# malani86/unet-DC-segmentation

Measured on AMD Instinct MI355X. Metric: images/sec fwd+bwd, 512x512x1 U-Net-DC, bs=8/GPU, higher is better.
Workload: dtype bf16

## Files before the change

unet_dc_segmentation_amd/csrc/igemm_conv.hip:

```cpp
#include <stdlib.h>

#include <stdio.h>

#include "kernels.h"

namespace unetdc {

template <typename T> struct Mma;
template <> struct Mma<bf16_t> {
  __device__ static __forceinline__ void run(f32x16& acc, const u32x4& a, const u32x4& b) {
    acc = __builtin_amdgcn_mfma_f32_32x32x16_bf16(__builtin_bit_cast(bf16x8, a), __builtin_bit_cast(bf16x8, b),
                                                  acc, 0, 0, 0);
  }
};
template <> struct Mma<float> {
  __device__ static __forceinline__ void run(f32x16& acc, const u32x4& a, const u32x4& b) {
#pragma unroll
    for (int s = 0; s < 4; ++s) {
      const unsigned int ua = a[s], ub = b[s];
      acc = __builtin_amdgcn_mfma_f32_32x32x2f32(bits_f32(ua), bits_f32(ub), acc, 0, 0, 0);
    }
  }
};

// ... 187 lines not shown
    }
  }
  if (p.mode == MODE_STATS) {
    s0 += __shfl_xor(s0, 32, 64); q0 += __shfl_xor(q0, 32, 64);
    s1 += __shfl_xor(s1, 32, 64); q1 += __shfl_xor(q1, 32, 64);
    float* red = reinterpret_cast<float*>(smem);
    if (h == 0) {
      red[(wave * 4 + 0) * 32 + r] = s0;
      red[(wave * 4 + 1) * 32 + r] = q0;
      red[(wave * 4 + 2) * 32 + r] = s1;
      red[(wave * 4 + 3) * 32 + r] = q1;
    }
    __syncthreads();
    if (tid < BN) {
      const int wn2 = tid >> 6, c2 = tid & 63, r2 = c2 >> 1, e = c2 & 1;
      float su = 0.f, sq = 0.f;
#pragma unroll
      for (int w2 = 0; w2 < WM; ++w2) {
        su += red[((w2 * WN + wn2) * 4 + e * 2 + 0) * 32 + r2];
        sq += red[((w2 * WN + wn2) * 4 + e * 2 + 1) * 32 + r2];
      }
      p.stats[((long)mblk * 2 + 0) * p.Cout + n0 + tid] = su;
      p.stats[((long)mblk * 2 + 1) * p.Cout + n0 + tid] = sq;
    }
  }
}

int igemm_mblocks(long M, int Cout) { (void)Cout; return ceil_div(M, 256); }

template <typename T, int WM, int WN>
static int launch_cfg(IgemmParams& p, hipStream_t stream) {
  constexpr int BM = 64 * WM, BN = 64 * WN;
  constexpr int LDS = 2 * (BM + BN) * 128;
  if (const int rc_ = ensure_dynamic_lds(reinterpret_cast<const void*>(&igemm_conv_kernel<T, WM, WN>), LDS, "igemm_conv_kernel")) return rc_;
  p.mblocks = ceil_div(p.M, BM);
  p.nblocks = p.Cout / BN;
  const long nwg = (long)p.mblocks * p.nblocks;
  hipLaunchKernelGGL((igemm_conv_kernel<T, WM, WN>), dim3((unsigned)nwg), dim3(256), LDS, stream, p);
  char nm[96];
  snprintf(nm, sizeof(nm), "igemm_conv_kernel<%s, %d, %d>", sizeof(T) == 2 ? "__bf16" : "float", WM, WN);
  note_kernel(nm);
  return check_launch("igemm_conv_kernel");
}

IgemmPlan plan_igemm(const IgemmParams& p, int dtype) {
  IgemmPlan pl{};
  const bool lattice = igemm_lattice_supported(p, dtype);
  if (p.in_scale) {
    if (lattice && p.mode == MODE_STATS && (p.Cout % 128 == 0 || p.Cin <= 256)) {
      pl.route = IGEMM_LATTICE;
      pl.writes_act = p.Cout % 128 == 0 && (long)p.M * p.Cin * 2 < (1L << 32);
    }
    return pl;
  }
  if (lattice) {
    pl.route = IGEMM_LATTICE;
    return pl;
  }
  if (igemm_halo_supported(p, dtype)) {
    pl.route = IGEMM_HALO;
    return pl;
  }
  const long es = dtype == UNETDC_BF16 ? 2 : 4;
  const long HoWo = (long)p.Ho * p.Wo;
  const long xbytes = (p.M / HoWo) * p.Hi * p.Wi * p.ldx * es;
  const long wbytes = (long)p.ntaps * p.Cout * p.Cin * es;
  const long opix = p.mode == MODE_SHUFFLE ? 4L * p.M : (long)p.M;
  const long obytes = opix * p.ldo * es, ybytes = p.mode == MODE_BNBWD ? (long)p.M * p.bn_ldy * es : 0;
  if (!(xbytes < (1L << 31) && wbytes < (1L << 31) && obytes < (1L << 32) && ybytes < (1L << 32) && p.M % HoWo == 0)) {
    pl.route = IGEMM_FIRSTGEN;
    pl.cfg = (p.Cout % 128 == 0) && p.mode != MODE_STATS;
    return pl;
  }
  const long blocks_a = (long)((p.M + 255) / 256) * (p.Cout / 256);
  const bool use_a = p.Cout % 256 == 0 && p.M >= 256 * 64 && blocks_a >= 200;
  const bool use_b = !use_a && p.Cout % 128 == 0;
  pl.route = IGEMM_DMA;
  pl.cfg = use_a ? 1 : (use_b ? 2 : 3);
  if (dtype == UNETDC_BF16 && p.M % 16 == 0 && !(p.mode == MODE_SHUFFLE && p.Wo % 16 != 0)) {
    pl.route = IGEMM_DMA16;
    const long blocks_b = (long)((p.M + 255) / 256) * (p.Cout / 128);
    if (pl.cfg == 2 && p.mode == MODE_SHUFFLE && p.Cout % 256 == 0 && blocks_a >= 200) pl.cfg = 1;
    else if (pl.cfg == 2 && blocks_b >= 100 && blocks_b < 200) pl.cfg = 3;
  }
  return pl;
}

int launch_igemm(IgemmParams& p, int dtype, hipStream_t stream) {
  const int esz = dtype == UNETDC_BF16 ? 2 : 4;
  const int ke = 128 / esz;
  UNETDC_REQUIRE(dtype == UNETDC_F32 || dtype == UNETDC_BF16, "igemm: bad dtype %d", dtype);
  UNETDC_REQUIRE(p.x && p.w && p.out, "igemm: null tensor pointer");
  UNETDC_REQUIRE(p.M > 0 && p.Cin > 0 && p.Cout > 0, "igemm: empty problem");
  UNETDC_REQUIRE(p.Cin % ke == 0, "igemm: Cin=%d must be a multiple of %d for this dtype", p.Cin, ke);
  UNETDC_REQUIRE(p.Cout % 64 == 0, "igemm: Cout=%d must be a multiple of 64", p.Cout);
  UNETDC_REQUIRE(p.ldx % (16 / esz) == 0 && p.ldo % (16 / esz) == 0, "igemm: ld not 16-byte aligned");
  UNETDC_REQUIRE(((uintptr_t)p.x % 16 == 0) && ((uintptr_t)p.w % 16 == 0) && ((uintptr_t)p.out % 16 == 0),
                 "igemm: pointers must be 16-byte aligned");
  UNETDC_REQUIRE(p.ntaps >= 1 && p.ntaps <= 9, "igemm: ntaps out of range");
  UNETDC_REQUIRE((long)p.M < (1L << 31) - 512, "igemm: too many pixels");
  if (p.mode == MODE_SHUFFLE) UNETDC_REQUIRE(p.shuf_c % 64 == 0, "igemm: convT channels must be a multiple of 64");
  if (p.mode == MODE_STATS) UNETDC_REQUIRE(p.stats != nullptr, "igemm: stats buffer missing");
  if (p.mode == MODE_AFFINE_RELU) UNETDC_REQUIRE(p.scale && p.shift, "igemm: scale/shift missing");
  if (p.mode == MODE_BNBWD)
    UNETDC_REQUIRE(p.stats && p.bn_y && p.scale && p.shift && p.bn_mean && p.bn_rstd, "igemm: BN-backward inputs missing");
  {
    const long howo = (long)p.Ho * p.Wo;
    const bool p2 = (p.Wo & (p.Wo - 1)) == 0 && (howo & (howo - 1)) == 0;
    p.wo_shift = p2 ? __builtin_ctz((unsigned)p.Wo) : -1;
    p.howo_shift = p2 ? __builtin_ctzl((unsigned long)howo) : -1;
  }
  const IgemmPlan pl = plan_igemm(p, dtype);
  switch (pl.route) {
    case IGEMM_LATTICE: return launch_igemm_lattice(p, stream);
    case IGEMM_HALO: return launch_igemm_halo(p, dtype, stream);
    case IGEMM_DMA: return launch_igemm_dma(p, pl.cfg, dtype, stream);
    case IGEMM_DMA16: return launch_igemm_dma16(p, pl.cfg, stream);
    case IGEMM_FIRSTGEN:
      if (p.mode == MODE_BNBWD) {
        set_error("igemm: the first-generation kernel has no fused BatchNorm-backward sums");
        return UNETDC_EUNSUPPORTED;
      }
      if (dtype == UNETDC_BF16) return pl.cfg ? launch_cfg<bf16_t, 2, 2>(p, stream) : launch_cfg<bf16_t, 4, 1>(p, stream);
      return pl.cfg ? launch_cfg<float, 2, 2>(p, stream) : launch_cfg<float, 4, 1>(p, stream);
  }
  set_error("igemm: input normalisation asked for a shape / configuration the lattice kernel does not take");
  return UNETDC_EUNSUPPORTED;
}

}
```

unet_dc_segmentation_amd/csrc/igemm_dma16.hip:

```cpp
#include <stdio.h>
#include <stdlib.h>

#include "igemm_epilogue16.h"
#include "kernels.h"
#include "lds_dma.h"

namespace unetdc {

#define LDS_PTR16(p) ((__attribute__((address_space(3))) void*)(p))
constexpr unsigned OOB16 = 0x80000000u;

template <int WM, int WN, int TMT, int NS>
__global__ __launch_bounds__(512, 2) void igemm_dma16_kernel(const IgemmParams p) {
#if defined(__HIP_DEVICE_COMPILE__)
  constexpr int NW = WM * WN;
  constexpr int BM = WM * TMT * 16, BN = WN * 64;
  constexpr int AI = BM / 8 / NW, BI = BN / 8 / NW;
  constexpr int ES = 2, KE = 64;
  constexpr int STAGE = (BM + BN) * 128;
  constexpr int PER = AI + BI;
  static_assert(BM % (8 * NW) == 0 && BN % (8 * NW) == 0, "tile/wave mismatch");
  static_assert(NS == 2 || NS == 3, "ring depth");
  static_assert((NS - 2) * PER <= 63, "vmcnt is a 6-bit counter");
  extern __shared__ __attribute__((aligned(16))) unsigned char smem[];

  const int tid = threadIdx.x, lane = tid & 63;
  const int wave = __builtin_amdgcn_readfirstlane(tid >> 6);
  const int wm = wave / WN, wn = wave % WN;
  const int tile = xcd_remap(blockIdx.x, gridDim.x);
  const int mblk = tile / p.nblocks, nblk = tile - mblk * p.nblocks;
  const int m0 = mblk * BM, n0 = nblk * BN;
  const int HoWo = p.Ho * p.Wo;
  const unsigned lds_base = lds_addr_of(smem);

  const unsigned xbytes = (unsigned)(((long)p.M / HoWo) * p.Hi * p.Wi * p.ldx * ES);
  const unsigned wbytes = (unsigned)((long)p.ntaps * p.Cout * p.Cin * ES);
  const __amdgpu_buffer_rsrc_t xr = __builtin_amdgcn_make_buffer_rsrc(const_cast<void*>(p.x), 0, xbytes, 0x00020000);
  const __amdgpu_buffer_rsrc_t wr = __builtin_amdgcn_make_buffer_rsrc(const_cast<void*>(p.w), 0, wbytes, 0x00020000);

  const bool p2 = p.wo_shift >= 0;
  const bool quad = p.quad_bpr > 0;
  auto decode = [&](int m, int& n, int& oy, int& ox) {
    if (quad) {
      const int blk = m >> 8, r = m & 255;
      n = blk / p.quad_bpi;
      const int b = blk - n * p.quad_bpi;
      const int qy = b / p.quad_bpr;
      oy = qy * 16 + (r >> 4);
      ox = (b - qy * p.quad_bpr) * 16 + (r & 15);
    } else if (p2) {
      n = m >> p.howo_shift;
      const int rem = m & (HoWo - 1);
      oy = rem >> p.wo_shift;
      ox = rem & (p.Wo - 1);
    } else {
      n = m / HoWo;
      const int rem = m - n * HoWo;
      oy = rem / p.Wo;
      ox = rem - oy * p.Wo;
    }
  };
  unsigned tapmask = 0;
  {
    int na, ya, xa, nb, yb, xb;
    const int mlast = (m0 + BM < p.M ? m0 + BM : p.M) - 1;
    decode(m0, na, ya, xa);
    decode(mlast, nb, yb, xb);
    int by0 = 0, by1 = p.Ho - 1, bx0 = 0, bx1 = p.Wo - 1;
    if (na == nb) {
      by0 = ya; by1 = yb;
      if (ya == yb || quad) { bx0 = xa; bx1 = xb; }
    }
    for (int t = 0; t < p.ntaps; ++t) {
      const int iy0 = by0 * p.stride + p.offy[t], iy1 = by1 * p.stride + p.offy[t];
      const int ix0 = bx0 * p.stride + p.offx[t], ix1 = bx1 * p.stride + p.offx[t];
      if (iy1 >= 0 && iy0 < p.Hi && ix1 >= 0 && ix0 < p.Wi) tapmask |= 1u << t;
    }
    tapmask = __builtin_amdgcn_readfirstlane(tapmask);
  }
  const int sub = lane >> 3, pc = lane & 7;
  int ys[AI], xs[AI];
  unsigned abase[AI];
#pragma unroll
  for (int j = 0; j < AI; ++j) {
    const int row = (wave + NW * j) * 8 + sub;
    const int m = m0 + row;
    const int c = pc ^ ((row >> 1) & 7);
    if (m < p.M) {
      int n, oy, ox;
      decode(m, n, oy, ox);
      ys[j] = oy * p.stride;
      xs[j] = ox * p.stride;
      abase[j] = (unsigned)(((n * p.Hi + ys[j]) * p.Wi + xs[j]) * p.ldx * ES + c * 16);
    } else {
      ys[j] = -(1 << 28);
      xs[j] = 0;
      abase[j] = 0;
    }
  }
  unsigned bbase[BI];
#pragma unroll
  for (int j = 0; j < BI; ++j) {
    const int lrow = (wave + NW * j) * 8 + sub;
    const int grp = lrow >> 6, q = lrow & 63;
    const int cc = (q & 15) * 4 + (q >> 4);
    const int c = pc ^ ((lrow >> 1) & 7);
    bbase[j] = (unsigned)((n0 + grp * 64 + cc) * p.Cin * ES + c * 16);
  }
  const int nkc = p.Cin / KE;
  const int nsteps = __popc(tapmask) * nkc;

  const int c16 = lane & 15, rb = lane >> 4;
  const int swz = (c16 >> 1) & 7;
  int a_rd[2], b_rd[2];
#pragma unroll
  for (int g = 0; g < 2; ++g) {
    const int ch = ((4 * g + rb) ^ swz) << 4;
    a_rd[g] = (wm * TMT * 16 + c16) * 128 + ch;
    b_rd[g] = BM * 128 + (wn * 64 + c16) * 128 + ch;
  }

  f32x4 acc[TMT][4];
#pragma unroll
  for (int i = 0; i < TMT; ++i)
#pragma unroll
    for (int j = 0; j < 4; ++j)
#pragma unroll
      for (int e = 0; e < 4; ++e) acc[i][j][e] = 0.f;

  int lt = 0, lkc = 0;
  while (lt < p.ntaps && !((tapmask >> lt) & 1u)) ++lt;

  auto issue = [&](int stage) {
    const int dy = p.offy[lt], dx = p.offx[lt];
    const unsigned dbytes = (unsigned)((dy * p.Wi + dx) * p.ldx * ES + lkc * 128);
    const unsigned sbase = lds_base + (unsigned)__builtin_amdgcn_readfirstlane(stage) * STAGE;
#pragma unroll
    for (int j = 0; j < AI; ++j) {
      const int iy = ys[j] + dy, ix = xs[j] + dx;
      const bool ok = (unsigned)iy < (unsigned)p.Hi && (unsigned)ix < (unsigned)p.Wi;
      lds_dma16(xr, sbase + (wave + NW * j) * 1024, ok ? abase[j] + dbytes : OOB16, 0u);
    }
    const unsigned wbytes_t = (unsigned)__builtin_amdgcn_readfirstlane((int)(lt * p.Cout * p.Cin * ES + lkc * 128));
#pragma unroll
    for (int j = 0; j < BI; ++j) lds_dma16(wr, sbase + BM * 128 + (wave + NW * j) * 1024, bbase[j], wbytes_t);
    do { ++lt; } while (lt < p.ntaps && !((tapmask >> lt) & 1u));
    if (lt >= p.ntaps) {
      ++lkc;
      lt = 0;
      while (lt < p.ntaps && !((tapmask >> lt) & 1u)) ++lt;
    }
  };

#pragma unroll
  for (int k = 0; k < NS - 1; ++k)
    if (k < nsteps) issue(k);
  const bool late = NS == 3 && wave >= NW / 2;
  int cur = 0, fill = NS - 1;
  for (int s = 0; s < nsteps; ++s) {
    if (NS > 2 && s + NS - 2 < nsteps) wait_vmcnt<(NS - 2) * PER>(); else wait_vmcnt<0>();
    raw_barrier();
    const bool more = s + NS - 1 < nsteps;
    const unsigned char* base = smem + cur * STAGE;
    {
      u32x4 fa[TMT], fb[2][4];
#pragma unroll
      for (int j = 0; j < 4; ++j) fb[0][j] = ld16(base + b_rd[0] + j * 16 * 128);
#pragma unroll
      for (int i = 0; i < TMT; ++i) fa[i] = ld16(base + a_rd[0] + i * 16 * 128);
#pragma unroll
      for (int j = 0; j < 4; ++j) fb[1][j] = ld16(base + b_rd[1] + j * 16 * 128);
      if (more && !late) issue(fill);
#pragma unroll
      for (int g = 0; g < 2; ++g)
#pragma unroll
        for (int i = 0; i < TMT; ++i) {
#pragma unroll
          for (int j = 0; j < 4; ++j)
            acc[i][j] = __builtin_amdgcn_mfma_f32_16x16x32_bf16(__builtin_bit_cast(bf16x8, fa[i]), __builtin_bit_cast(bf16x8, fb[g][j]),
                                                                acc[i][j], 0, 0, 0);
          if (g == 0) {
            fa[i] = ld16(base + a_rd[1] + i * 16 * 128);
            __builtin_amdgcn_sched_barrier(0);
          }
        }
    }
    if (more && late) issue(fill);
    cur = cur + 1 == NS ? 0 : cur + 1;
    fill = fill + 1 == NS ? 0 : fill + 1;
  }

  const int col = n0 + wn * 64 + 4 * c16;
  const unsigned ldob = (unsigned)(p.ldo * ES), ldyb = (unsigned)(p.bn_ldy * ES);
  bool tile_ok[TMT];
  unsigned voff[TMT], yoff[TMT];
  int ccol = col;
  unsigned row_bytes = ldob;
  if (p.mode == MODE_SHUFFLE) {
    const int ab = col / p.shuf_c;
    ccol = col - ab * p.shuf_c;
    row_bytes = 2 * ldob;
#pragma unroll
    for (int i = 0; i < TMT; ++i) {
      const int mb = m0 + (wm * TMT + i) * 16;
      tile_ok[i] = mb < p.M;
      int n, oy, ox;
      decode(mb, n, oy, ox);
      const unsigned pix = (unsigned)((n * 2 * p.Ho + 2 * oy + (ab >> 1)) * (2 * p.Wo) + 2 * ox + (ab & 1));
      voff[i] = (pix + 8u * rb) * ldob + (unsigned)(ccol * ES);
      yoff[i] = 0;
    }
  } else {
#pragma unroll
    for (int i = 0; i < TMT; ++i) {
      const int mb = m0 + (wm * TMT + i) * 16;
      tile_ok[i] = mb < p.M;
      int pix = mb;
      if (quad) {
        int n, oy, ox;
        decode(mb, n, oy, ox);
        pix = (n * p.Ho + oy) * p.Wo + ox;
      }
      voff[i] = (unsigned)(pix + 4 * rb) * ldob + (unsigned)(col * ES);
      yoff[i] = (unsigned)(pix + 4 * rb) * ldyb + (unsigned)(col * ES);
    }
  }
  float s4[4] = {0.f, 0.f, 0.f, 0.f}, q4[4] = {0.f, 0.f, 0.f, 0.f};
  switch (p.mode) {
    case MODE_STATS: epilogue16<MODE_STATS, TMT>(p, acc, tile_ok, voff, row_bytes, yoff, ldyb, ccol, s4, q4); break;
    case MODE_AFFINE_RELU: epilogue16<MODE_AFFINE_RELU, TMT>(p, acc, tile_ok, voff, row_bytes, yoff, ldyb, ccol, s4, q4); break;
    case MODE_BNBWD: epilogue16<MODE_BNBWD, TMT>(p, acc, tile_ok, voff, row_bytes, yoff, ldyb, ccol, s4, q4); break;
    default: epilogue16<MODE_STORE, TMT>(p, acc, tile_ok, voff, row_bytes, yoff, ldyb, ccol, s4, q4); break;
  }
  if (p.mode == MODE_STATS || p.mode == MODE_BNBWD) write_stat_rows16<WM, WN>(p, smem, s4, q4, mblk, n0, tid, wave, c16, rb);
#endif
}

template <int WM, int WN, int TMT, int NS>
static int launch_dma16_cfg(IgemmParams& p, hipStream_t stream) {
  constexpr int BM = WM * TMT * 16, BN = WN * 64;
  constexpr int LDS = NS * (BM + BN) * 128;
  static_assert(LDS <= 160 * 1024, "ring does not fit");
  if (const int rc_ = ensure_dynamic_lds(reinterpret_cast<const void*>(&igemm_dma16_kernel<WM, WN, TMT, NS>), LDS, "igemm_dma16_kernel")) return rc_;
  p.mblocks = ceil_div(p.M, BM);
  p.nblocks = p.Cout / BN;
  p.quad_bpr = p.quad_bpi = 0;
  if (BM == 256 && p.ntaps == 9 && p.stride == 1 && p.mode != MODE_SHUFFLE && p.Ho == p.Hi && p.Wo == p.Wi &&
      p.offy[8] >= 16 && p.offy[8] % 16 == 0 && p.offx[8] == p.offy[8] && p.Ho % 16 == 0 && p.Wo % 16 == 0 &&
      p.M % ((long)p.Ho * p.Wo) == 0) {
    p.quad_bpr = p.Wo / 16;
    p.quad_bpi = (p.Ho / 16) * p.quad_bpr;
  }
  const long nwg = (long)p.mblocks * p.nblocks;
  hipLaunchKernelGGL((igemm_dma16_kernel<WM, WN, TMT, NS>), dim3((unsigned)nwg), dim3(WM * WN * 64), LDS, stream, p);
  char nm[96];
  snprintf(nm, sizeof(nm), "igemm_dma16_kernel<%d, %d, %d>%s%s", WM, WN, TMT, NS == 3 ? " ring3" : "", p.quad_bpr ? " blocks16x16" : "");
  note_kernel(nm);
  return check_launch("igemm_dma16_kernel");
}

int launch_igemm_dma16(IgemmParams& p, int cfg, hipStream_t stream) {
  if (cfg == 1) return launch_dma16_cfg<2, 4, 8, 2>(p, stream);
  if (cfg == 2) return launch_dma16_cfg<4, 2, 4, 3>(p, stream);
  return launch_dma16_cfg<4, 1, 4, 2>(p, stream);
}

}
```

unet_dc_segmentation_amd/csrc/kernels.h:

```cpp
#pragma once
#include <algorithm>
#include <type_traits>

#include "common.h"
#include "workspace.h"
#include "../../include/unetdc_hip.h"

namespace unetdc {

enum { MODE_STORE = 0, MODE_STATS = 1, MODE_AFFINE_RELU = 2, MODE_SHUFFLE = 3, MODE_BNBWD = 4 };
#define UNETDC_EUNSUPPORTED (-4)

struct IgemmParams {
  const void* x;
  const void* w;
  void* out;
  const float* bias;
  const float* scale;
  const float* shift;
  float* stats;
  const void* bn_y;
  const float* bn_mean;
  const float* bn_rstd;
  int bn_ldy;
  int M, Ho, Wo, Hi, Wi, Cin, Cout, ldx, ldo, ntaps, stride, mode, shuf_c;
  int mblocks, nblocks;
  int wo_shift, howo_shift;
  int quad_bpr, quad_bpi;
  const float* in_scale;
  const float* in_shift;
  void* act_out;
  int ld_act;
  int offy[9];
  int offx[9];
};
enum IgemmRoute {
  IGEMM_UNSUPPORTED = 0,
  IGEMM_LATTICE,
  IGEMM_HALO,
  IGEMM_DMA,
  IGEMM_DMA16,
  IGEMM_FIRSTGEN,
};
struct IgemmPlan {
  int route;
  int cfg;
  bool writes_act;
};
IgemmPlan plan_igemm(const IgemmParams& p, int dtype);
int launch_igemm(IgemmParams& p, int dtype, hipStream_t stream);
int igemm_mblocks(long M, int Cout);
bool igemm_lattice_supported(const IgemmParams& p, int dtype);
bool igemm_halo_supported(const IgemmParams& p, int dtype);
int launch_igemm_lattice(IgemmParams& p, hipStream_t stream);
int launch_igemm_halo(IgemmParams& p, int dtype, hipStream_t stream);
int launch_igemm_dma(IgemmParams& p, int cfg, int dtype, hipStream_t stream);
int launch_igemm_dma16(IgemmParams& p, int cfg, hipStream_t stream);

struct WgradParams {
  const void* a;
  const void* b;
  float* part;
  int N, H, W, Hb, Wb, CI, CJ, lda, ldb, ntaps, stride;
  int P;
  int chunk;
  int ksplit, itiles, jtiles;
  int adv_y, adv_x;
  int offy[9];
  int offx[9];
  const float* in_scale;
  const float* in_shift;
};
enum WgradRoute {
  WGRAD_UNSUPPORTED = 0,
  WGRAD_CONVT,
  WGRAD_RECT,
  WGRAD_FUSED,
  WGRAD_DMA,
  WGRAD_LEGACY,
};
struct WgradFusedPlan {
  bool supported;
  bool paired;
  bool bnin;
  int pf;
  int ysplit, rows_per_unit, imgs_per_unit, half_lds;
  int threads, nwg;
  int lds, lds_attr;
  int units;
  long workspace;
};
struct WgradPlan {
  int route;
  WgradFusedPlan fused;
  int ksplit;
  int chunk, tw, step;
  int steps_per_half;
  long workspace;
};
WgradPlan plan_wgrad(const WgradParams& p, int dtype);
long wgrad_workspace_bound(int N, int H, int W, int CI, int CJ, int ntaps, int dtype);
int launch_wgrad(WgradParams& p, float* out, void* workspace, long workspace_bytes, int dtype, hipStream_t stream);
bool convt_wgrad_split(int N, int H, int W, int CI, int CJ, int& ksplit, int& steps_per_half);
int launch_convt_wgrad_fused(const WgradParams& w, const WgradPlan& pl, hipStream_t stream);
int wgrad_rect_units(int N, int H, int W, int CI, int CJ, int d);
int launch_wgrad_rect(const WgradParams& w, const WgradPlan& pl, float* out, hipStream_t stream);
WgradFusedPlan plan_wgrad_fused(const WgradParams& w, int dtype);
long wgrad_fused_workspace_bytes(int N, int H, int W, int CI, int CJ, int dtype);
int launch_wgrad_fused(const WgradParams& w, const WgradFusedPlan& pl, int dtype, hipStream_t stream);
int wgrad_dma_tile(int CI, int CJ);
int wgrad_dma_pixel_step(int dtype, int tw);
int launch_wgrad_dma_kernel(WgradParams& p, int tw, int dtype, hipStream_t stream);

struct FirstParams {
  const float* x;
  const float* w;
  const float* bias;
  const float* scale;
  const float* shift;
  void* y;
  float* stats;
  int N, H, W, Cin, Cout, ldy, dil;
};
struct FirstWgradParams {
  const float* x;
  const void* dy;
  float* part;
  int N, H, W, Cin, Cout, lddy, dil;
  const void* bn_y; int bn_ldy;
  const float* bn_scale; const float* bn_shift; const float* bn_mean; const float* bn_rstd; const float* bn_k;
};
struct FirstPlan {
  bool mfma;
  int fwd_blocks;
  bool wgrad_mfma;
  int wgrad_blocks;
  int rows_blocks;
  long workspace;
};
FirstPlan plan_first(long P, int Cin, int Cout);
// ... 197 lines not shown
```

Measured before the change: 784.8.

## Add persistent dma16 igemm kernel that overlaps epilogue with next tile's loads

```diff
diff --git a/unet_dc_segmentation_amd/csrc/igemm_conv.hip b/unet_dc_segmentation_amd/csrc/igemm_conv.hip
--- a/unet_dc_segmentation_amd/csrc/igemm_conv.hip
+++ b/unet_dc_segmentation_amd/csrc/igemm_conv.hip
@@ -293,6 +293,8 @@
     const long blocks_b = (long)((p.M + 255) / 256) * (p.Cout / 128);
     if (pl.cfg == 2 && p.mode == MODE_SHUFFLE && p.Cout % 256 == 0 && blocks_a >= 200) pl.cfg = 1;
     else if (pl.cfg == 2 && blocks_b >= 100 && blocks_b < 200) pl.cfg = 3;
+    const long nblocks = p.Cout / (pl.cfg == 1 ? 256 : (pl.cfg == 2 ? 128 : 64)), grid = dma16_persistent_grid(pl.cfg);
+    pl.persistent = grid > 0 && (long)((p.M + 255) / 256) * nblocks > grid && (grid / 8) % nblocks == 0 && p.ntaps * (p.Cin / 64) <= 4;
   }
   return pl;
 }
@@ -326,7 +328,7 @@
     case IGEMM_LATTICE: return launch_igemm_lattice(p, stream);
     case IGEMM_HALO: return launch_igemm_halo(p, dtype, stream);
     case IGEMM_DMA: return launch_igemm_dma(p, pl.cfg, dtype, stream);
-    case IGEMM_DMA16: return launch_igemm_dma16(p, pl.cfg, stream);
+    case IGEMM_DMA16: return launch_igemm_dma16(p, pl.cfg, pl.persistent, stream);
     case IGEMM_FIRSTGEN:
       if (p.mode == MODE_BNBWD) {
         set_error("igemm: the first-generation kernel has no fused BatchNorm-backward sums");
diff --git a/unet_dc_segmentation_amd/csrc/igemm_dma16.hip b/unet_dc_segmentation_amd/csrc/igemm_dma16.hip
--- a/unet_dc_segmentation_amd/csrc/igemm_dma16.hip
+++ b/unet_dc_segmentation_amd/csrc/igemm_dma16.hip
@@ -7,26 +7,275 @@
 
 namespace unetdc {
 
-#define LDS_PTR16(p) ((__attribute__((address_space(3))) void*)(p))
 constexpr unsigned OOB16 = 0x80000000u;
+constexpr int DMA16_LDS_PER_CU = 160 * 1024;
+
+template <int WM, int WN, int TMT, int NS>
+struct Dma16Tile {
+  static constexpr int NW = WM * WN;
+  static constexpr int BM = WM * TMT * 16, BN = WN * 64;
+  static constexpr int AI = BM / 8 / NW, BI = BN / 8 / NW;
+  static constexpr int ES = 2, KE = 64;
+  static constexpr int STAGE = (BM + BN) * 128;
+  static constexpr int PER = AI + BI;
+  static constexpr int RING = NS * STAGE;
+  static constexpr int RED = NW * 128 * 4;
+  static constexpr int KC = NW * 1024;
+  static constexpr int LDS_PERSISTENT = RING + RED + KC;
+  static constexpr bool CAN_PERSIST = NW == 8 && NS == 3 && LDS_PERSISTENT <= DMA16_LDS_PER_CU;
+  static constexpr int EST = TMT * 4;
+  static_assert(BM % (8 * NW) == 0 && BN % (8 * NW) == 0, "tile/wave mismatch");
+  static_assert(NS == 2 || NS == 3, "ring depth");
+  static_assert((NS - 2) * PER + EST <= 63, "vmcnt is a 6-bit counter");
+  static_assert(RING <= DMA16_LDS_PER_CU, "ring does not fit");
+};
+
+#if defined(__HIP_DEVICE_COMPILE__)
+__device__ __forceinline__ void dma16_decode(const IgemmParams& p, int m, int& n, int& oy, int& ox) {
+  const int HoWo = p.Ho * p.Wo;
+  if (p.quad_bpr > 0) {
+    const int blk = m >> 8, r = m & 255;
+    n = blk / p.quad_bpi;
+    const int b = blk - n * p.quad_bpi;
+    const int qy = b / p.quad_bpr;
+    oy = qy * 16 + (r >> 4);
+    ox = (b - qy * p.quad_bpr) * 16 + (r & 15);
+  } else if (p.wo_shift >= 0) {
+    n = m >> p.howo_shift;
+    const int rem = m & (HoWo - 1);
+    oy = rem >> p.wo_shift;
+    ox = rem & (p.Wo - 1);
+  } else {
+    n = m / HoWo;
+    const int rem = m - n * HoWo;
+    oy = rem / p.Wo;
+    ox = rem - oy * p.Wo;
+  }
+}
+
+template <int BM>
+__device__ __forceinline__ unsigned dma16_tapmask(const IgemmParams& p, int m0) {
+  unsigned tapmask = 0;
+  int na, ya, xa, nb, yb, xb;
+  const int mlast = (m0 + BM < p.M ? m0 + BM : p.M) - 1;
+  dma16_decode(p, m0, na, ya, xa);
+  dma16_decode(p, mlast, nb, yb, xb);
+  int by0 = 0, by1 = p.Ho - 1, bx0 = 0, bx1 = p.Wo - 1;
+  if (na == nb) {
+    by0 = ya; by1 = yb;
+    if (ya == yb || p.quad_bpr > 0) { bx0 = xa; bx1 = xb; }
+  }
+  for (int t = 0; t < p.ntaps; ++t) {
+    const int iy0 = by0 * p.stride + p.offy[t], iy1 = by1 * p.stride + p.offy[t];
+    const int ix0 = bx0 * p.stride + p.offx[t], ix1 = bx1 * p.stride + p.offx[t];
+    if (iy1 >= 0 && iy0 < p.Hi && ix1 >= 0 && ix0 < p.Wi) tapmask |= 1u << t;
+  }
+  return (unsigned)__builtin_amdgcn_readfirstlane((int)tapmask);
+}
+
+__device__ __forceinline__ int dma16_first_tap(const IgemmParams& p, unsigned tapmask) {
+  int lt = 0;
+  while (lt < p.ntaps && !((tapmask >> lt) & 1u)) ++lt;
+  return lt;
+}
+
+template <int AI, int BI>
+struct Dma16Rows {
+  int ys[AI], xs[AI];
+  unsigned abase[AI], bbase[BI];
+};
+
+template <typename T>
+__device__ __forceinline__ void dma16_rows(const IgemmParams& p, int m0, int n0, int wave, int lane, Dma16Rows<T::AI, T::BI>& r) {
+  const int sub = lane >> 3, pc = lane & 7;
+#pragma unroll
+  for (int j = 0; j < T::AI; ++j) {
+    const int row = (wave + T::NW * j) * 8 + sub;
+    const int m = m0 + row;
+    const int c = pc ^ ((row >> 1) & 7);
+    if (m < p.M) {
+      int n, oy, ox;
+      dma16_decode(p, m, n, oy, ox);
+      r.ys[j] = oy * p.stride;
+      r.xs[j] = ox * p.stride;
+      r.abase[j] = (unsigned)(((n * p.Hi + r.ys[j]) * p.Wi + r.xs[j]) * p.ldx * T::ES + c * 16);
+    } else {
+      r.ys[j] = -(1 << 28);
+      r.xs[j] = 0;
+      r.abase[j] = 0;
+    }
+  }
+#pragma unroll
+  for (int j = 0; j < T::BI; ++j) {
+    const int lrow = (wave + T::NW * j) * 8 + sub;
+    const int grp = lrow >> 6, q = lrow & 63;
+    const int cc = (q & 15) * 4 + (q >> 4);
+    const int c = pc ^ ((lrow >> 1) & 7);
+    r.bbase[j] = (unsigned)((n0 + grp * 64 + cc) * p.Cin * T::ES + c * 16);
+  }
+}
+
+template <typename T>
+__device__ __forceinline__ void dma16_issue_stage(const IgemmParams& p, __amdgpu_buffer_rsrc_t xr, __amdgpu_buffer_rsrc_t wr,
+                                                  const Dma16Rows<T::AI, T::BI>& r, int wave, unsigned sbase, unsigned tapmask,
+                                                  int& lt, int& lkc) {
+  const int dy = p.offy[lt], dx = p.offx[lt];
+  const unsigned dbytes = (unsigned)((dy * p.Wi + dx) * p.ldx * T::ES + lkc * 128);
+#pragma unroll
+  for (int j = 0; j < T::AI; ++j) {
+    const int iy = r.ys[j] + dy, ix = r.xs[j] + dx;
+    const bool ok = (unsigned)iy < (unsigned)p.Hi && (unsigned)ix < (unsigned)p.Wi;
+    lds_dma16(xr, sbase + (wave + T::NW * j) * 1024, ok ? r.abase[j] + dbytes : OOB16, 0u);
+  }
+  const unsigned wbytes_t = (unsigned)__builtin_amdgcn_readfirstlane((int)(lt * p.Cout * p.Cin * T::ES + lkc * 128));
+#pragma unroll
+  for (int j = 0; j < T::BI; ++j) lds_dma16(wr, sbase + T::BM * 128 + (wave + T::NW * j) * 1024, r.bbase[j], wbytes_t);
+  do { ++lt; } while (lt < p.ntaps && !((tapmask >> lt) & 1u));
+  if (lt >= p.ntaps) {
+    ++lkc;
+    lt = dma16_first_tap(p, tapmask);
+  }
+}
+
+template <int TMT, typename Mid>
+__device__ __forceinline__ void dma16_mfma_step(const unsigned char* base, const int (&a_rd)[2], const int (&b_rd)[2],
+                                                f32x4 (&acc)[TMT][4], Mid&& mid) {
+  u32x4 fa[TMT], fb[2][4];
+#pragma unroll
+  for (int j = 0; j < 4; ++j) fb[0][j] = ld16(base + b_rd[0] + j * 16 * 128);
+#pragma unroll
+  for (int i = 0; i < TMT; ++i) fa[i] = ld16(base + a_rd[0] + i * 16 * 128);
+#pragma unroll
+  for (int j = 0; j < 4; ++j) fb[1][j] = ld16(base + b_rd[1] + j * 16 * 128);
+  mid();
+#pragma unroll
+  for (int g = 0; g < 2; ++g)
+#pragma unroll
+    for (int i = 0; i < TMT; ++i) {
+#pragma unroll
+      for (int j = 0; j < 4; ++j)
+        acc[i][j] = __builtin_amdgcn_mfma_f32_16x16x32_bf16(__builtin_bit_cast(bf16x8, fa[i]), __builtin_bit_cast(bf16x8, fb[g][j]),
+                                                            acc[i][j], 0, 0, 0);
+      if (g == 0) {
+        fa[i] = ld16(base + a_rd[1] + i * 16 * 128);
+        __builtin_amdgcn_sched_barrier(0);
+      }
+    }
+}
+
+template <int TMT>
+__device__ __forceinline__ void dma16_zero(f32x4 (&acc)[TMT][4]) {
+#pragma unroll
+  for (int i = 0; i < TMT; ++i)
+#pragma unroll
+    for (int j = 0; j < 4; ++j)
+#pragma unroll
+      for (int e = 0; e < 4; ++e) acc[i][j][e] = 0.f;
+}
+
+template <int WN>
+__device__ __forceinline__ Epi16Consts dma16_consts(const IgemmParams& p, int n0, int wave, int lane) {
+  const int col = n0 + (wave % WN) * 64 + 4 * (lane & 15);
+  const int ccol = p.mode == MODE_SHUFFLE ? col % p.shuf_c : col;
+  switch (p.mode) {
+    case MODE_AFFINE_RELU: return epi16_consts<MODE_AFFINE_RELU>(p, ccol);
+    case MODE_BNBWD: return epi16_consts<MODE_BNBWD>(p, ccol);
+    default: return epi16_consts<MODE_STORE>(p, ccol);
+  }
+}
+
+template <int TMT>
+__device__ __forceinline__ void dma16_store_tiles(const IgemmParams& p, f32x4 (&acc)[TMT][4], const bool (&tile_ok)[TMT],
+                                                  const unsigned (&voff)[TMT], unsigned row_bytes, const unsigned (&yoff)[TMT],
+                                                  unsigned ldyb, const Epi16Consts& kc, float (&s4)[4], float (&q4)[4]) {
+  switch (p.mode) {
+    case MODE_STATS: epilogue16c<MODE_STATS, TMT>(p, acc, tile_ok, voff, row_bytes, yoff, ldyb, kc, s4, q4); break;
+    case MODE_AFFINE_RELU: epilogue16c<MODE_AFFINE_RELU, TMT>(p, acc, tile_ok, voff, row_bytes, yoff, ldyb, kc, s4, q4); break;
+    case MODE_BNBWD: epilogue16c<MODE_BNBWD, TMT>(p, acc, tile_ok, voff, row_bytes, yoff, ldyb, kc, s4, q4); break;
+    default: epilogue16c<MODE_STORE, TMT>(p, acc, tile_ok, voff, row_bytes, yoff, ldyb, kc, s4, q4); break;
+  }
+}
+
+template <int WM, int WN, int TMT, bool PRELOADED>
+__device__ __forceinline__ void dma16_epilogue(const IgemmParams& p, f32x4 (&acc)[TMT][4], const Epi16Consts& kc, unsigned char* red,
+                                               int mblk, int n0, int tid, int wave, int lane) {
+  constexpr int ES = 2, BM = WM * TMT * 16;
+  const int wm = wave / WN, wn = wave % WN;
+  const int c16 = lane & 15, rb = lane >> 4;
+  const int m0 = mblk * BM;
+  const int col = n0 + wn * 64 + 4 * c16;
+  const unsigned ldob = (unsigned)(p.ldo * ES), ldyb = (unsigned)(p.bn_ldy * ES);
+  bool tile_ok[TMT];
+  unsigned voff[TMT], yoff[TMT];
+  unsigned row_bytes = ldob;
+  if (p.mode == MODE_SHUFFLE) {
+    const int ab = col / p.shuf_c;
+    const int ccol = col - ab * p.shuf_c;
+    row_bytes = 2 * ldob;
+#pragma unroll
+    for (int i = 0; i < TMT; ++i) {
+      const int mb = m0 + (wm * TMT + i) * 16;
+      tile_ok[i] = mb < p.M;
+      int n, oy, ox;
+      dma16_decode(p, mb, n, oy, ox);
+      const unsigned pix = (unsigned)((n * 2 * p.Ho + 2 * oy + (ab >> 1)) * (2 * p.Wo) + 2 * ox + (ab & 1));
+      voff[i] = (pix + 8u * rb) * ldob + (unsigned)(ccol * ES);
+      yoff[i] = 0;
+    }
+  } else {
+#pragma unroll
+    for (int i = 0; i < TMT; ++i) {
+      const int mb = m0 + (wm * TMT + i) * 16;
+      tile_ok[i] = mb < p.M;
+      int pix = mb;
+      if (p.quad_bpr > 0) {
+        int n, oy, ox;
+        dma16_decode(p, mb, n, oy, ox);
+        pix = (n * p.Ho + oy) * p.Wo + ox;
+      }
+      voff[i] = (unsigned)(pix + 4 * rb) * ldob + (unsigned)(col * ES);
+      yoff[i] = (unsigned)(pix + 4 * rb) * ldyb + (unsigned)(col * ES);
+    }
+  }
+  float s4[4] = {0.f, 0.f, 0.f, 0.f}, q4[4] = {0.f, 0.f, 0.f, 0.f};
+  if (!PRELOADED) {
+    const Epi16Consts k1 = dma16_consts<WN>(p, n0, wave, lane);
+    dma16_store_tiles<TMT>(p, acc, tile_ok, voff, row_bytes, yoff, ldyb, k1, s4, q4);
+  } else if (m0 + BM <= p.M) {
+    bool all_ok[TMT];
+#pragma unroll
+    for (int i = 0; i < TMT; ++i) all_ok[i] = true;
+    dma16_store_tiles<TMT>(p, acc, all_ok, voff, row_bytes, yoff, ldyb, kc, s4, q4);
+  } else {
+    dma16_store_tiles<TMT>(p, acc, tile_ok, voff, row_bytes, yoff, ldyb, kc, s4, q4);
+    __builtin_amdgcn_s_waitcnt(0x0F70);
+  }
+  if (p.mode == MODE_STATS || p.mode == MODE_BNBWD) write_stat_rows16<WM, WN>(p, red, s4, q4, mblk, n0, tid, wave, c16, rb);
+}
+
+template <typename T, int WN, int TMT>
+__device__ __forceinline__ void dma16_fragment_offsets(int wave, int lane, int (&a_rd)[2], int (&b_rd)[2]) {
+  const int wm = wave / WN, wn = wave % WN;
+  const int c16 = lane & 15, rb = lane >> 4;
+  const int swz = (c16 >> 1) & 7;
+#pragma unroll
+  for (int g = 0; g < 2; ++g) {
+    const int ch = ((4 * g + rb) ^ swz) << 4;
+    a_rd[g] = (wm * TMT * 16 + c16) * 128 + ch;
+    b_rd[g] = T::BM * 128 + (wn * 64 + c16) * 128 + ch;
+  }
+}
+#endif
 
 template <int WM, int WN, int TMT, int NS>
 __global__ __launch_bounds__(512, 2) void igemm_dma16_kernel(const IgemmParams p) {
 #if defined(__HIP_DEVICE_COMPILE__)
-  constexpr int NW = WM * WN;
-  constexpr int BM = WM * TMT * 16, BN = WN * 64;
-  constexpr int AI = BM / 8 / NW, BI = BN / 8 / NW;
-  constexpr int ES = 2, KE = 64;
-  constexpr int STAGE = (BM + BN) * 128;
-  constexpr int PER = AI + BI;
-  static_assert(BM % (8 * NW) == 0 && BN % (8 * NW) == 0, "tile/wave mismatch");
-  static_assert(NS == 2 || NS == 3, "ring depth");
-  static_assert((NS - 2) * PER <= 63, "vmcnt is a 6-bit counter");
+  using T = Dma16Tile<WM, WN, TMT, NS>;
+  constexpr int NW = T::NW, BM = T::BM, BN = T::BN, ES = T::ES, KE = T::KE, STAGE = T::STAGE, PER = T::PER;
   extern __shared__ __attribute__((aligned(16))) unsigned char smem[];
 
   const int tid = threadIdx.x, lane = tid & 63;
   const int wave = __builtin_amdgcn_readfirstlane(tid >> 6);
-  const int wm = wave / WN, wn = wave % WN;
   const int tile = xcd_remap(blockIdx.x, gridDim.x);
   const int mblk = tile / p.nblocks, nblk = tile - mblk * p.nblocks;
   const int m0 = mblk * BM, n0 = nblk * BN;
@@ -38,118 +287,22 @@
   const __amdgpu_buffer_rsrc_t xr = __builtin_amdgcn_make_buffer_rsrc(const_cast<void*>(p.x), 0, xbytes, 0x00020000);
   const __amdgpu_buffer_rsrc_t wr = __builtin_amdgcn_make_buffer_rsrc(const_cast<void*>(p.w), 0, wbytes, 0x00020000);
 
-  const bool p2 = p.wo_shift >= 0;
-  const bool quad = p.quad_bpr > 0;
-  auto decode = [&](int m, int& n, int& oy, int& ox) {
-    if (quad) {
-      const int blk = m >> 8, r = m & 255;
-      n = blk / p.quad_bpi;
-      const int b = blk - n * p.quad_bpi;
-      const int qy = b / p.quad_bpr;
-      oy = qy * 16 + (r >> 4);
-      ox = (b - qy * p.quad_bpr) * 16 + (r & 15);
-    } else if (p2) {
-      n = m >> p.howo_shift;
-      const int rem = m & (HoWo - 1);
-      oy = rem >> p.wo_shift;
-      ox = rem & (p.Wo - 1);
-    } else {
-      n = m / HoWo;
-      const int rem = m - n * HoWo;
-      oy = rem / p.Wo;
-      ox = rem - oy * p.Wo;
-    }
-  };
-  unsigned tapmask = 0;
-  {
-    int na, ya, xa, nb, yb, xb;
-    const int mlast = (m0 + BM < p.M ? m0 + BM : p.M) - 1;
-    decode(m0, na, ya, xa);
-    decode(mlast, nb, yb, xb);
-    int by0 = 0, by1 = p.Ho - 1, bx0 = 0, bx1 = p.Wo - 1;
-    if (na == nb) {
-      by0 = ya; by1 = yb;
-      if (ya == yb || quad) { bx0 = xa; bx1 = xb; }
-    }
-    for (int t = 0; t < p.ntaps; ++t) {
-      const int iy0 = by0 * p.stride + p.offy[t], iy1 = by1 * p.stride + p.offy[t];
-      const int ix0 = bx0 * p.stride + p.offx[t], ix1 = bx1 * p.stride + p.offx[t];
-      if (iy1 >= 0 && iy0 < p.Hi && ix1 >= 0 && ix0 < p.Wi) tapmask |= 1u << t;
-    }
-    tapmask = __builtin_amdgcn_readfirstlane(tapmask);
-  }
-  const int sub = lane >> 3, pc = lane & 7;
-  int ys[AI], xs[AI];
-  unsigned abase[AI];
-#pragma unroll
-  for (int j = 0; j < AI; ++j) {
-    const int row = (wave + NW * j) * 8 + sub;
-    const int m = m0 + row;
-    const int c = pc ^ ((row >> 1) & 7);
-    if (m < p.M) {
-      int n, oy, ox;
-      decode(m, n, oy, ox);
-      ys[j] = oy * p.stride;
-      xs[j] = ox * p.stride;
-      abase[j] = (unsigned)(((n * p.Hi + ys[j]) * p.Wi + xs[j]) * p.ldx * ES + c * 16);
-    } else {
-      ys[j] = -(1 << 28);
-      xs[j] = 0;
-      abase[j] = 0;
-    }
-  }
-  unsigned bbase[BI];
-#pragma unroll
-  for (int j = 0; j < BI; ++j) {
-    const int lrow = (wave + NW * j) * 8 + sub;
-    const int grp = lrow >> 6, q = lrow & 63;
-    const int cc = (q & 15) * 4 + (q >> 4);
-    const int c = pc ^ ((lrow >> 1) & 7);
-    bbase[j] = (unsigned)((n0 + grp * 64 + cc) * p.Cin * ES + c * 16);
-  }
+  const unsigned tapmask = dma16_tapmask<BM>(p, m0);
+  Dma16Rows<T::AI, T::BI> rows;
+  dma16_rows<T>(p, m0, n0, wave, lane, rows);
   const int nkc = p.Cin / KE;
   const int nsteps = __popc(tapmask) * nkc;
 
-  const int c16 = lane & 15, rb = lane >> 4;
-  const int swz = (c16 >> 1) & 7;
   int a_rd[2], b_rd[2];
-#pragma unroll
-  for (int g = 0; g < 2; ++g) {
-    const int ch = ((4 * g + rb) ^ swz) << 4;
-    a_rd[g] = (wm * TMT * 16 + c16) * 128 + ch;
-    b_rd[g] = BM * 128 + (wn * 64 + c16) * 128 + ch;
-  }
+  dma16_fragment_offsets<T, WN, TMT>(wave, lane, a_rd, b_rd);
 
   f32x4 acc[TMT][4];
-#pragma unroll
-  for (int i = 0; i < TMT; ++i)
-#pragma unroll
-    for (int j = 0; j < 4; ++j)
-#pragma unroll
-      for (int e = 0; e < 4; ++e) acc[i][j][e] = 0.f;
-
-  int lt = 0, lkc = 0;
-  while (lt < p.ntaps && !((tapmask >> lt) & 1u)) ++lt;
-
+  dma16_zero<TMT>(acc);
+
+  int lt = dma16_first_tap(p, tapmask), lkc = 0;
   auto issue = [&](int stage) {
-    const int dy = p.offy[lt], dx = p.offx[lt];
-    const unsigned dbytes = (unsigned)((dy * p.Wi + dx) * p.ldx * ES + lkc * 128);
     const unsigned sbase = lds_base + (unsigned)__builtin_amdgcn_readfirstlane(stage) * STAGE;
-#pragma unroll
-    for (int j = 0; j < AI; ++j) {
-      const int iy = ys[j] + dy, ix = xs[j] + dx;
-      const bool ok = (unsigned)iy < (unsigned)p.Hi && (unsigned)ix < (unsigned)p.Wi;
-      lds_dma16(xr, sbase + (wave + NW * j) * 1024, ok ? abase[j] + dbytes : OOB16, 0u);
-    }
-    const unsigned wbytes_t = (unsigned)__builtin_amdgcn_readfirstlane((int)(lt * p.Cout * p.Cin * ES + lkc * 128));
-#pragma unroll
-    for (int j = 0; j < BI; ++j) lds_dma16(wr, sbase + BM * 128 + (wave + NW * j) * 1024, bbase[j], wbytes_t);
-    do { ++lt; } while (lt < p.ntaps && !((tapmask >> lt) & 1u));
-    if (lt >= p.ntaps) {
-      ++lkc;
-      lt = 0;
-      while (lt < p.ntaps && !((tapmask >> lt) & 1u)) ++lt;
-    }
+    dma16_issue_stage<T>(p, xr, wr, rows, wave, sbase, tapmask, lt, lkc);
   };
 
 #pragma unroll
@@ -161,108 +314,188 @@
     if (NS > 2 && s + NS - 2 < nsteps) wait_vmcnt<(NS - 2) * PER>(); else wait_vmcnt<0>();
     raw_barrier();
     const bool more = s + NS - 1 < nsteps;
-    const unsigned char* base = smem + cur * STAGE;
-    {
-      u32x4 fa[TMT], fb[2][4];
-#pragma unroll
-      for (int j = 0; j < 4; ++j) fb[0][j] = ld16(base + b_rd[0] + j * 16 * 128);
-#pragma unroll
-      for (int i = 0; i < TMT; ++i) fa[i] = ld16(base + a_rd[0] + i * 16 * 128);
-#pragma unroll
-      for (int j = 0; j < 4; ++j) fb[1][j] = ld16(base + b_rd[1] + j * 16 * 128);
-      if (more && !late) issue(fill);
-#pragma unroll
-      for (int g = 0; g < 2; ++g)
-#pragma unroll
-        for (int i = 0; i < TMT; ++i) {
-#pragma unroll
-          for (int j = 0; j < 4; ++j)
-            acc[i][j] = __builtin_amdgcn_mfma_f32_16x16x32_bf16(__builtin_bit_cast(bf16x8, fa[i]), __builtin_bit_cast(bf16x8, fb[g][j]),
-                                                                acc[i][j], 0, 0, 0);
-          if (g == 0) {
-            fa[i] = ld16(base + a_rd[1] + i * 16 * 128);
-            __builtin_amdgcn_sched_barrier(0);
-          }
-        }
-    }
+    dma16_mfma_step<TMT>(smem + cur * STAGE, a_rd, b_rd, acc, [&]() { if (more && !late) issue(fill); });
     if (more && late) issue(fill);
     cur = cur + 1 == NS ? 0 : cur + 1;
     fill = fill + 1 == NS ? 0 : fill + 1;
   }
 
-  const int col = n0 + wn * 64 + 4 * c16;
-  const unsigned ldob = (unsigned)(p.ldo * ES), ldyb = (unsigned)(p.bn_ldy * ES);
-  bool tile_ok[TMT];
-  unsigned voff[TMT], yoff[TMT];
-  int ccol = col;
-  unsigned row_bytes = ldob;
-  if (p.mode == MODE_SHUFFLE) {
-    const int ab = col / p.shuf_c;
-    ccol = col - ab * p.shuf_c;
-    row_bytes = 2 * ldob;
-#pragma unroll
-    for (int i = 0; i < TMT; ++i) {
-      const int mb = m0 + (wm * TMT + i) * 16;
-      tile_ok[i] = mb < p.M;
-      int n, oy, ox;
-      decode(mb, n, oy, ox);
-      const unsigned pix = (unsigned)((n * 2 * p.Ho + 2 * oy + (ab >> 1)) * (2 * p.Wo) + 2 * ox + (ab & 1));
-      voff[i] = (pix + 8u * rb) * ldob + (unsigned)(ccol * ES);
-      yoff[i] = 0;
-    }
-  } else {
-#pragma unroll
-    for (int i = 0; i < TMT; ++i) {
-      const int mb = m0 + (wm * TMT + i) * 16;
-      tile_ok[i] = mb < p.M;
-      int pix = mb;
-      if (quad) {
-        int n, oy, ox;
-        decode(mb, n, oy, ox);
-        pix = (n * p.Ho + oy) * p.Wo + ox;
-      }
-      voff[i] = (unsigned)(pix + 4 * rb) * ldob + (unsigned)(col * ES);
-      yoff[i] = (unsigned)(pix + 4 * rb) * ldyb + (unsigned)(col * ES);
-    }
-  }
-  float s4[4] = {0.f, 0.f, 0.f, 0.f}, q4[4] = {0.f, 0.f, 0.f, 0.f};
-  switch (p.mode) {
-    case MODE_STATS: epilogue16<MODE_STATS, TMT>(p, acc, tile_ok, voff, row_bytes, yoff, ldyb, ccol, s4, q4); break;
-    case MODE_AFFINE_RELU: epilogue16<MODE_AFFINE_RELU, TMT>(p, acc, tile_ok, voff, row_bytes, yoff, ldyb, ccol, s4, q4); break;
-    case MODE_BNBWD: epilogue16<MODE_BNBWD, TMT>(p, acc, tile_ok, voff, row_bytes, yoff, ldyb, ccol, s4, q4); break;
-    default: epilogue16<MODE_STORE, TMT>(p, acc, tile_ok, voff, row_bytes, yoff, ldyb, ccol, s4, q4); break;
-  }
-  if (p.mode == MODE_STATS || p.mode == MODE_BNBWD) write_stat_rows16<WM, WN>(p, smem, s4, q4, mblk, n0, tid, wave, c16, rb);
+  dma16_epilogue<WM, WN, TMT, false>(p, acc, Epi16Consts{}, smem, mblk, n0, tid, wave, lane);
 #endif
 }
 
 template <int WM, int WN, int TMT, int NS>
-static int launch_dma16_cfg(IgemmParams& p, hipStream_t stream) {
-  constexpr int BM = WM * TMT * 16, BN = WN * 64;
-  constexpr int LDS = NS * (BM + BN) * 128;
-  static_assert(LDS <= 160 * 1024, "ring does not fit");
-  if (const int rc_ = ensure_dynamic_lds(reinterpret_cast<const void*>(&igemm_dma16_kernel<WM, WN, TMT, NS>), LDS, "igemm_dma16_kernel")) return rc_;
-  p.mblocks = ceil_div(p.M, BM);
-  p.nblocks = p.Cout / BN;
+__global__ __launch_bounds__(512, 2) void igemm_dma16_persistent_kernel(const IgemmParams p) {
+#if defined(__HIP_DEVICE_COMPILE__)
+  using T = Dma16Tile<WM, WN, TMT, NS>;
+  constexpr int NW = T::NW, BM = T::BM, BN = T::BN, ES = T::ES, KE = T::KE, STAGE = T::STAGE, PER = T::PER, EST = T::EST;
+  extern __shared__ __attribute__((aligned(16))) unsigned char smem[];
+
+  const int tid = threadIdx.x, lane = tid & 63;
+  const int wave = __builtin_amdgcn_readfirstlane(tid >> 6);
+  const int HoWo = p.Ho * p.Wo;
+  const unsigned lds_base = lds_addr_of(smem);
+  const int nitems = p.mblocks * p.nblocks, G = gridDim.x;
+
+  const unsigned xbytes = (unsigned)(((long)p.M / HoWo) * p.Hi * p.Wi * p.ldx * ES);
+  const unsigned wbytes = (unsigned)((long)p.ntaps * p.Cout * p.Cin * ES);
+  const __amdgpu_buffer_rsrc_t xr = __builtin_amdgcn_make_buffer_rsrc(const_cast<void*>(p.x), 0, xbytes, 0x00020000);
+  const __amdgpu_buffer_rsrc_t wr = __builtin_amdgcn_make_buffer_rsrc(const_cast<void*>(p.w), 0, wbytes, 0x00020000);
+  const int nkc = p.Cin / KE;
+
+  int a_rd[2], b_rd[2];
+  dma16_fragment_offsets<T, WN, TMT>(wave, lane, a_rd, b_rd);
+
+  f32x4 acc[TMT][4];
+  dma16_zero<TMT>(acc);
+
+  auto fresh_lane = [&]() {
+    int l = lane;
+    asm volatile("" : "+v"(l));
+    return l;
+  };
+
+  Dma16Rows<T::AI, T::BI> rows;
+  unsigned mask_i = 0;
+  int lt = 0, lkc = 0, rem_i = 0, it_i = blockIdx.x, gi = 0, fill = 0;
+  auto prepare = [&]() {
+    while (rem_i == 0 && it_i < nitems) {
+      const int tile = xcd_remap(it_i, nitems);
+      const int mblk = tile / p.nblocks, nblk = tile - mblk * p.nblocks;
+      mask_i = dma16_tapmask<BM>(p, mblk * BM);
+      dma16_rows<T>(p, mblk * BM, nblk * BN, wave, fresh_lane(), rows);
+      rem_i = __popc(mask_i) * nkc;
+      lt = dma16_first_tap(p, mask_i);
+      lkc = 0;
+      it_i += G;
+    }
+  };
+  auto issue_next = [&]() {
+    if (rem_i == 0) return;
+    const unsigned sbase = lds_base + (unsigned)__builtin_amdgcn_readfirstlane(fill) * STAGE;
+    dma16_issue_stage<T>(p, xr, wr, rows, wave, sbase, mask_i, lt, lkc);
+    --rem_i;
+    ++gi;
+    fill = fill + 1 == NS ? 0 : fill + 1;
+  };
+
+  const bool late = NS == 3 && wave >= NW / 2;
+  int g = 0, cur = 0, s = 0, it = blockIdx.x, mblk = 0, nblk = 0, nsteps = 0;
+  bool pend = false, pend_full = false, epi_counts = false;
+  int pend_mblk = 0, pend_nblk = 0, epi_gi = 0;
+  auto open_item = [&]() {
+    if (it >= nitems) return;
+    const int tile = xcd_remap(it, nitems);
+    mblk = tile / p.nblocks;
+    nblk = tile - mblk * p.nblocks;
+    nsteps = __popc(dma16_tapmask<BM>(p, mblk * BM)) * nkc;
+  };
+  open_item();
+#pragma nounroll
+  for (int k = 0; k < NS - 1; ++k) {
+    prepare();
+    issue_next();
+  }
+  float* kc_lds = reinterpret_cast<float*>(smem + T::RING + T::RED + wave * 1024 + (lane & 15) * 64);
+  {
+    const Epi16Consts c = dma16_consts<WN>(p, nblk * BN, wave, lane);
+#pragma unroll
+    for (int k = 0; k < 4; ++k) { kc_lds[k] = c.k0[k]; kc_lds[4 + k] = c.k1[k]; kc_lds[8 + k] = c.mu[k]; kc_lds[12 + k] = c.rs[k]; }
+  }
+  const bool epi_first = p.mode == MODE_BNBWD;
+
+  for (;;) {
+    const bool done = it >= nitems;
+    const bool step = !done && s < nsteps;
+    prepare();
+    if (step) {
+      const bool ahead = NS > 2 && gi - 1 - g == NS - 2;
+      const bool epi = epi_counts && g < epi_gi;
+      if (ahead) { if (epi) wait_vmcnt<(NS - 2) * PER + EST>(); else wait_vmcnt<(NS - 2) * PER>(); }
+      else { if (epi) wait_vmcnt<EST>(); else wait_vmcnt<0>(); }
+      raw_barrier();
+    }
+    bool issued = false;
+    if (pend && s == 0) {
+      if (step && !epi_first && !late) { issue_next(); issued = true; }
+      Epi16Consts kc;
+#pragma unroll
+      for (int k = 0; k < 4; ++k) { kc.k0[k] = kc_lds[k]; kc.k1[k] = kc_lds[4 + k]; kc.mu[k] = kc_lds[8 + k]; kc.rs[k] = kc_lds[12 + k]; }
+      const int el = fresh_lane();
+      dma16_epilogue<WM, WN, TMT, true>(p, acc, kc, smem + T::RING, pend_mblk, pend_nblk * BN, wave * 64 + el, wave, el);
+      epi_counts = pend_full;
+      epi_gi = gi;
+      dma16_zero<TMT>(acc);
+      pend = false;
+    }
+    if (done) break;
+    if (step) {
+      dma16_mfma_step<TMT>(smem + cur * STAGE, a_rd, b_rd, acc, [&]() { if (!late && !issued) issue_next(); });
+      if (late) issue_next();
+      cur = cur + 1 == NS ? 0 : cur + 1;
+      ++g;
+      ++s;
+    }
+    if (s == nsteps) {
+      pend = true;
+      pend_mblk = mblk;
+      pend_nblk = nblk;
+      pend_full = (mblk + 1) * BM <= p.M;
+      it += G;
+      s = 0;
+      open_item();
+    }
+  }
+#endif
+}
+
+constexpr int DMA16_PERSISTENT_GRID = 256;
+
+template <int WM, int WN, int TMT, int NS>
+static int launch_dma16_cfg(IgemmParams& p, bool persistent, hipStream_t stream) {
+  using T = Dma16Tile<WM, WN, TMT, NS>;
+  p.mblocks = ceil_div(p.M, T::BM);
+  p.nblocks = p.Cout / T::BN;
   p.quad_bpr = p.quad_bpi = 0;
-  if (BM == 256 && p.ntaps == 9 && p.stride == 1 && p.mode != MODE_SHUFFLE && p.Ho == p.Hi && p.Wo == p.Wi &&
+  if (T::BM == 256 && p.ntaps == 9 && p.stride == 1 && p.mode != MODE_SHUFFLE && p.Ho == p.Hi && p.Wo == p.Wi &&
       p.offy[8] >= 16 && p.offy[8] % 16 == 0 && p.offx[8] == p.offy[8] && p.Ho % 16 == 0 && p.Wo % 16 == 0 &&
       p.M % ((long)p.Ho * p.Wo) == 0) {
     p.quad_bpr = p.Wo / 16;
     p.quad_bpi = (p.Ho / 16) * p.quad_bpr;
   }
-  const long nwg = (long)p.mblocks * p.nblocks;
-  hipLaunchKernelGGL((igemm_dma16_kernel<WM, WN, TMT, NS>), dim3((unsigned)nwg), dim3(WM * WN * 64), LDS, stream, p);
-  char nm[96];
-  snprintf(nm, sizeof(nm), "igemm_dma16_kernel<%d, %d, %d>%s%s", WM, WN, TMT, NS == 3 ? " ring3" : "", p.quad_bpr ? " blocks16x16" : "");
+  const long items = (long)p.mblocks * p.nblocks;
+  if constexpr (T::CAN_PERSIST) {
+    if (persistent) {
+      if (items <= DMA16_PERSISTENT_GRID || (DMA16_PERSISTENT_GRID / 8) % p.nblocks != 0) {
+        set_error("igemm_dma16: persistent form asked for %ld items in %d n-blocks (plan_igemm)", items, p.nblocks);
+        return UNETDC_ELAUNCH;
+      }
+      if (const int rc_ = ensure_dynamic_lds(reinterpret_cast<const void*>(&igemm_dma16_persistent_kernel<WM, WN, TMT, NS>),
+                                             T::LDS_PERSISTENT, "igemm_dma16_persistent_kernel")) return rc_;
+      hipLaunchKernelGGL((igemm_dma16_persistent_kernel<WM, WN, TMT, NS>), dim3(DMA16_PERSISTENT_GRID), dim3(T::NW * 64),
+                         T::LDS_PERSISTENT, stream, p);
+    }
+  } else if (persistent) {
+    set_error("igemm_dma16: this tile has no persistent form (plan_igemm)");
+    return UNETDC_ELAUNCH;
+  }
+  if (!persistent) {
+    if (const int rc_ = ensure_dynamic_lds(reinterpret_cast<const void*>(&igemm_dma16_kernel<WM, WN, TMT, NS>), T::RING, "igemm_dma16_kernel")) return rc_;
+    hipLaunchKernelGGL((igemm_dma16_kernel<WM, WN, TMT, NS>), dim3((unsigned)items), dim3(T::NW * 64), T::RING, stream, p);
+  }
+  char nm[112];
+  snprintf(nm, sizeof(nm), "igemm_dma16_kernel<%d, %d, %d>%s%s%s", WM, WN, TMT, NS == 3 ? " ring3" : "", p.quad_bpr ? " blocks16x16" : "",
+           persistent ? " persistent" : "");
   note_kernel(nm);
   return check_launch("igemm_dma16_kernel");
 }
 
-int launch_igemm_dma16(IgemmParams& p, int cfg, hipStream_t stream) {
-  if (cfg == 1) return launch_dma16_cfg<2, 4, 8, 2>(p, stream);
-  if (cfg == 2) return launch_dma16_cfg<4, 2, 4, 3>(p, stream);
-  return launch_dma16_cfg<4, 1, 4, 2>(p, stream);
-}
-
-}
+int dma16_persistent_grid(int cfg) { return cfg == 2 ? DMA16_PERSISTENT_GRID : 0; }
+
+int launch_igemm_dma16(IgemmParams& p, int cfg, bool persistent, hipStream_t stream) {
+  if (cfg == 1) return launch_dma16_cfg<2, 4, 8, 2>(p, persistent, stream);
+  if (cfg == 2) return launch_dma16_cfg<4, 2, 4, 3>(p, persistent, stream);
+  return launch_dma16_cfg<4, 1, 4, 2>(p, persistent, stream);
+}
+
+}
diff --git a/unet_dc_segmentation_amd/csrc/kernels.h b/unet_dc_segmentation_amd/csrc/kernels.h
--- a/unet_dc_segmentation_amd/csrc/kernels.h
+++ b/unet_dc_segmentation_amd/csrc/kernels.h
@@ -45,6 +45,7 @@
 struct IgemmPlan {
   int route;
   int cfg;
+  bool persistent;
   bool writes_act;
 };
 IgemmPlan plan_igemm(const IgemmParams& p, int dtype);
@@ -55,7 +56,8 @@
 int launch_igemm_lattice(IgemmParams& p, hipStream_t stream);
 int launch_igemm_halo(IgemmParams& p, int dtype, hipStream_t stream);
 int launch_igemm_dma(IgemmParams& p, int cfg, int dtype, hipStream_t stream);
-int launch_igemm_dma16(IgemmParams& p, int cfg, hipStream_t stream);
+int launch_igemm_dma16(IgemmParams& p, int cfg, bool persistent, hipStream_t stream);
+int dma16_persistent_grid(int cfg);
 
 struct WgradParams {
   const void* a;
```

Result: no change. 783.0 (-0.2%).
